# efeslab/Atom

Measured on AMD Instinct MI355X. Metric: effective TOPS, W4A4 group-128 GEMM + 128 INT8 outlier cols, fp16 out, higher is better.
Workload: dtype int4xint4 exact integer dot (BF6-coded on the f8f6f4 MFMA; INT8 MFMA for the keeper), fp32 dequant, fp16 out

## Files before the change

atom_amd/_lib.py:

```python
from __future__ import annotations

import ctypes
import os
import subprocess

_HERE = os.path.dirname(os.path.abspath(__file__))
LIB_PATH = os.path.join(_HERE, "libatom_hip.so")
CSRC = os.path.join(_HERE, "csrc")

OK = 0
ERR_INVALID_ARG, ERR_SHAPE, ERR_ALIGN, ERR_LAUNCH = -22, -33, -14, -5
SCALE_LAYOUT_REF = 0
SCALE_LAYOUT_PLAIN = 1
QUANT_KERNEL = 0
QUANT_SIM = 1
QUANT_WIDE_CODES = 0x100
A_WIDE = 0x100
QUANT_F6_CODES = 0x200
AB_F6 = 0x200
O4_REF_EXTREMA = 0x800
B_F6S = 0x400
WS_WEIGHT_CACHED = 0x1000
B_SCALE_PAIRS = 0x2000
WS_VERIFY = 0x4000
Q_REORDER, Q_RMSNORM, Q_ADD_RMSNORM, Q_SILU_MUL = 1, 2, 3, 4
KV_STEP_OVERFLOW, KV_STEP_BAD_LENGTH = 1, 2
KV_BEAM_BAD_PARENT, KV_BEAM_BAD_PAGE = 4, 8
GUIDE_FREE, GUIDE_DEAD = -1, -2
GUIDE_REJECTED, GUIDE_BAD_STATE = 1, 2
F6_PITCH = 104

_vp = ctypes.c_void_p
_i64 = ctypes.c_int64
_int = ctypes.c_int
_f32 = ctypes.c_float

SIGNATURES = {
    "atom_version": (ctypes.c_char_p, []),
    "atom_strerror": (ctypes.c_char_p, [_int]),
    "atom_scale_size": (ctypes.c_size_t, [_i64, _int]),
    "atom_gemm_w4a4_f16": (_int, [_vp] * 9 + [_i64, _i64, _i64, _int, _int, _int, _vp]),
    "atom_gemm_w4a4_workspace_bytes": (ctypes.c_size_t, [_i64, _i64, _i64]),
    "atom_gemm_w4a4_ws_recodes": (_int, [_i64, _i64, _i64]),
    "atom_gemm_w4a4_ws_recodes_cached": (_int, [_i64, _i64, _i64]),
    "atom_gemm_w4a4_packed_order": (_int, [_i64, _i64, _i64, _int]),
    "atom_check_scale_pairs": (_int, [_vp, _i64, _i64, _vp, _vp]),
    "atom_verify_weight_f6s": (_int, [_vp, _vp, _i64, _i64, _vp, _vp, _vp]),
    "atom_gemm_w4a4_f16_ws": (_int, [_vp] * 9 + [_i64, _i64, _i64, _int, _int, _int, _vp, ctypes.c_size_t, _vp]),
    "atom_gemm_w4a4_multi_fits": (_int, [_i64, _i64, _int, _i64]),
    "atom_gemm_w4a4_multi": (_int, [_vp] * 11 + [ctypes.c_uint, _vp, _i64, _i64, _int, _i64, _int, _int, _int, _vp]),
    "atom_gemm_w4a4_multi_q_fits": (_int, [_int, _i64, _i64, _int, _i64]),
    "atom_gemm_w4a4_multi_q": (_int, [_int] + [_vp] * 5 + [_f32, _f32] + [_vp] * 7 + [ctypes.c_uint, _vp, _i64, _i64, _int, _i64, _int, _int, _vp]),
    "atom_gemm_w4a4_o4": (_int, [_vp] * 10 + [_i64, _i64, _i64, _int, _int, _int, _vp]),
    "atom_gemm_w4a4_o4_workspace_bytes": (ctypes.c_size_t, [_i64, _i64, _i64]),
    "atom_gemm_w4a4_o4_ws": (_int, [_vp] * 10 + [_i64, _i64, _i64, _int, _int, _int, _vp, ctypes.c_size_t, _vp]),
    "atom_reorder_quant_f16": (_int, [_vp, _vp, _i64, _int, _int, _f32, _int, _vp, _vp, _vp, _vp, _vp, _vp]),
    "atom_rmsnorm_reorder_quant_f16": (_int, [_vp, _vp, _f32, _vp, _i64, _int, _int, _f32, _int,
                                              _vp, _vp, _vp, _vp, _vp, _vp]),
    "atom_add_rmsnorm_reorder_quant_f16": (_int, [_vp, _vp, _vp, _vp, _f32, _vp, _i64, _int, _int, _f32, _int,
                                                  _vp, _vp, _vp, _vp, _vp, _vp]),
    "atom_silu_mul_quant_f16": (_int, [_vp, _vp, _i64, _int, _int, _f32, _int, _vp, _vp, _vp, _vp, _vp, _vp]),
    "atom_quant_weight_w4": (_int, [_vp, _i64, _i64, _f32, _int, _vp, _vp, _vp, _vp, _vp, _vp]),
    "atom_pack_weight_w4": (_int, [_vp, _i64, _i64, _int, _vp, _vp, _vp, _vp, _vp, _vp]),
    "atom_f6_rows": (ctypes.c_size_t, [_i64]),
    "atom_repack_weight_f6": (_int, [_vp, _i64, _i64, _vp, _vp]),
    "atom_repack_act_f6": (_int, [_vp, _vp, _i64, _i64, _int, _vp, _vp]),
    "atom_f6_weight_bytes": (ctypes.c_size_t, [_i64, _i64]),
    "atom_gemm_w4a4_f6_order": (ctypes.c_int, [_i64, _i64, _i64]),
    "atom_repack_weight_f6s": (_int, [_vp, _vp, _i64, _i64, _vp, _vp]),
    "atom_kv_fake_quant_f16": (_int, [_vp, _vp, _i64, _int, _i64, _i64, _i64, _i64, _int, _f32, _vp]),
    "atom_kv_append_i4": (_int, [_vp] * 10 + [_i64] + [_int] * 6 + [_vp]),
    "atom_kv_quant_append_f32": (_int, [_vp] * 7 + [_int] * 6 + [_vp]),
    "atom_gemm_w4a4_f32": (_int, [_vp] * 9 + [_i64, _i64, _i64, _int, _int, _int, _vp]),
    "atom_gemm_w4a4_silu_mul_quant_f6": (_int, [_vp] * 6 + [_i64, _i64, _i64, _int, _int, _int, _f32, _int] + [_vp] * 6),
    "atom_batch_decode_i4_workspace_bytes": (ctypes.c_size_t, [_int, _int, _int, _int]),
    "atom_batch_decode_i4_splits": (_int, [_int, _int, _int, _int]),
    "atom_gemm_w4a4_multi_merge_q_fits": (_int, [_i64, _i64, _int, _i64, _int]),
    "atom_gemm_w4a4_multi_merge_q": (_int, [_vp, _int, _vp, _f32] + [_vp] * 7 + [ctypes.c_uint, _vp, _i64, _i64, _int, _i64, _int, _int, _vp]),
    "atom_batch_decode_i4": (_int, [_vp] * 7 + [_int] * 6 + [_f32, _f32, _int, _vp, ctypes.c_size_t, _vp]),
    "atom_batch_decode_append_i4": (_int, [_vp] * 9 + [_int] * 6 + [_f32, _f32, _int, _vp, ctypes.c_size_t, _vp]),
    "atom_batch_prefill_i4_workspace_bytes": (ctypes.c_size_t, [_i64, _int, _int, _int, _int, _int]),
    "atom_batch_prefill_i4": (_int, [_vp, _vp, _vp, _i64, _int] + [_vp] * 5 + [_int] * 6 + [_f32, _f32, _int, _vp, ctypes.c_size_t, _vp]),
    "atom_batch_decode_gqa_i4_workspace_bytes": (ctypes.c_size_t, [_int] * 5),
    "atom_batch_decode_gqa_i4_splits": (_int, [_int] * 5),
    "atom_batch_decode_gqa_i4": (_int, [_vp] * 7 + [_int] * 7 + [_f32, _f32, _int, _vp, ctypes.c_size_t, _vp]),
    "atom_batch_prefill_gqa_i4_workspace_bytes": (ctypes.c_size_t, [_i64] + [_int] * 6),
    "atom_batch_prefill_gqa_i4": (_int, [_vp, _vp, _vp, _i64, _int] + [_vp] * 5 + [_int] * 7 + [_f32, _f32, _int, _vp, ctypes.c_size_t, _vp]),
    "atom_kv_step_i4": (_int, [_vp] * 7 + [_int] * 4 + [_vp]),
    "atom_moe_max_tiles": (_i64, [_i64, _int]),
    "atom_moe_route_topk": (_int, [_vp, _i64, _int, _int] + [_vp] * 9),
    "atom_moe_gemm_w4a4_f16": (_int, [_vp] * 15 + [_i64, _i64, _int, _i64, _int, _i64, _int, _int, _int, _vp]),
# ... 66 lines not shown
```

atom_amd/csrc/common.h:

```cpp
#pragma once
#include <hip/hip_runtime.h>
#include <stdint.h>
#include <atomic>

#include "../../include/atom_hip.h"

#ifdef ATOM_TOOLS
#include <cstdlib>
#define ATOM_TUNE(name, dflt) ([]() -> int { const char *e = getenv(name); return e ? atoi(e) : (dflt); }())
#else
#define ATOM_TUNE(name, dflt) (dflt)
#endif

namespace atom {

constexpr int kGroup = 128;
constexpr int kKeeper = 128;

typedef _Float16 half_t;
typedef int v4i __attribute__((ext_vector_type(4)));
typedef int v16i __attribute__((ext_vector_type(16)));
typedef float v4f __attribute__((ext_vector_type(4)));
typedef unsigned int v4u __attribute__((ext_vector_type(4)));
typedef unsigned int v2u __attribute__((ext_vector_type(2)));
// ... 25 lines not shown
  float clip;
  int ref_layout;
};

struct GemmParams {
  const uint8_t *A4, *B4;
  const half_t *sA, *sB;
  const uint8_t *A8, *B8;
  const half_t *sA8, *sB8;
  half_t *D;
  uint8_t *D4;
  half_t *Dsz;
  float *ws;
  int splits;
  int M, N;
  int K4h;
  int G;
  int ref_layout;
  int a_wide;
  int64_t ldA;
  int64_t f6_rows_a, f6_rows_b;
  int o4_ref;
  int b_pairs;
  GateUpOut gu;
  const float *sB32;
  void *seg_out[3];
  const half_t *seg_add;
  int seg_n;
  unsigned seg_f32;
  int q_op;
  const half_t *q_x, *q_x2;
  const half_t *q_res;
  half_t *q_res_out;
  const int16_t *q_idx;
  float q_eps, q_clip;
  int q_roles;
  const float *q_part;
  int q_splits;
};

int launch_gemm_v2(const GemmParams &p, int ns, hipStream_t s);
int launch_gemm_v2_o4(const GemmParams &p, hipStream_t s);
int launch_gemm_v3(const GemmParams &p, int cfg, hipStream_t s);
int launch_gemv(const GemmParams &p, hipStream_t s);
#ifdef ATOM_TOOLS
constexpr int kGemvMaxTokens = 8;
#else
constexpr int kGemvMaxTokens = 2;
#endif
int launch_gemv1(const GemmParams &p, hipStream_t s);
int launch_gemv1_f32(const GemmParams &p, hipStream_t s);
int launch_gemv1_multi(const GemmParams &p, hipStream_t s);
int launch_gemm_skinny(const GemmParams &p, hipStream_t s);
int launch_gemm_skinny_f32(const GemmParams &p, hipStream_t s);
int launch_gemm_skinny_o4(const GemmParams &p, hipStream_t s);
int launch_gemm_skinny_multi(const GemmParams &p, hipStream_t s);
bool skinny_q_fits(int q_op, int64_t M, int64_t K_total);
int launch_gemm_skinny_multi_q(const GemmParams &p, hipStream_t s);
bool gemvq_fits(int q_op, int64_t M, int64_t N, int64_t K_total);
bool gemvq_merge_fits(int64_t M, int64_t N, int64_t K_total, int splits);
int launch_gemvq_multi_q(const GemmParams &p, hipStream_t s);
enum F6Cfg : int {
  F6_256x256 = 0, F6_128x128 = 3, F6_128x128_KG2 = 6, F6_256x128 = 8, F6_MID = 20,
  F6_256x128_P = 1, F6_64x128 = 2, F6_128x128_8W = 4, F6_128x128_KG2_S2 = 5, F6_64x128_KG2 = 9, F6_256x256_32 = 10, F6_64x128_KG4 = 12, F6_128x128_32 = 13, F6_256x256_P = 30,
};
inline int f6_cfg_order(int cfg) { return cfg == F6_64x128_KG4 ? 4 : ((cfg == F6_128x128_KG2_S2 || cfg == F6_128x128_KG2 || cfg == F6_64x128_KG2) ? 2 : 1); }
int launch_gemm_f6(const GemmParams &p, int cfg, hipStream_t s);
int launch_gemm_f6_mid(const GemmParams &p, hipStream_t s);
int launch_gemm_mid(const GemmParams &p, hipStream_t s);
int launch_gemm_f6_gateup(const GemmParams &p, int sim, hipStream_t s);

int launch_repack_f6(const uint8_t *src, int64_t rows, int K4h, int G, const half_t *scale, int64_t ld, int ref_layout,
                     uint8_t *out, hipStream_t s);
int launch_repack_f6_pair(const uint8_t *A4, int64_t M, const half_t *sA, int64_t ldA, int ref_layout, uint8_t *outA,
                          const half_t *sB, float *sB32,
                          const uint8_t *B4, int64_t N, uint8_t *outB, int K4h, int G, hipStream_t s);

int launch_check_scale_pairs(const half_t *sB, int64_t G, int64_t N, int32_t *n_bad, hipStream_t s);
int launch_verify_weight_f6s(const uint8_t *B4, const half_t *sB, int64_t N, int K4h, int G, const uint8_t *have, int32_t *n_bad, hipStream_t s);

template <int BYTES>
__device__ __forceinline__ void lds_dma(const void *gsrc, const void *lds_dst) {
  static_assert(BYTES == 16 || BYTES == 4 || BYTES == 2, "LDS-DMA piece size");
  const unsigned m0v = __builtin_amdgcn_readfirstlane((unsigned)(size_t)(const __attribute__((address_space(3))) char *)lds_dst);
  if constexpr (BYTES == 16) asm volatile("s_mov_b32 m0, %0\n\ts_nop 0\n\tglobal_load_lds_dwordx4 %1, off" ::"s"(m0v), "v"(gsrc) : "memory");
  else if constexpr (BYTES == 4) asm volatile("s_mov_b32 m0, %0\n\ts_nop 0\n\tglobal_load_lds_dword %1, off" ::"s"(m0v), "v"(gsrc) : "memory");
// ... 81 lines not shown
```

atom_amd/csrc/gemm_w4a4.hip:

```cpp
#include "common.h"

using namespace atom;

static bool shape_ok(int64_t M, int64_t N, int64_t K_total, bool n64) {
  return M >= 1 && N >= 64 && (!n64 || (N % 64) == 0) && K_total >= 256 && ((K_total - kKeeper) % kGroup) == 0;
}
static bool segments_ok(int64_t M, int64_t N_seg, int nseg, int64_t K_total) {
  return M >= 1 && nseg >= 1 && nseg <= 3 && N_seg >= 16 && (N_seg % 16) == 0 && K_total >= 256 && ((K_total - kKeeper) % kGroup) == 0;
}

static void fill_dims(GemmParams &p, int64_t M, int64_t N, int64_t K_total, int scale_layout, bool f6, bool f6s) {
  p.M = (int)M; p.N = (int)N;
  p.K4h = (int)((K_total - kKeeper) / 2); p.G = (int)((K_total - kKeeper) / kGroup);
  p.ref_layout = scale_layout == ATOM_SCALE_LAYOUT_REF;
  p.f6_rows_a = f6 ? (M + 255) / 256 * 256 : 0;
  p.f6_rows_b = f6 ? (N + 255) / 256 * 256 : 0;
  p.sB32 = f6s ? reinterpret_cast<const float *>(p.B4 + (size_t)p.G * (size_t)p.f6_rows_b * 104) : nullptr;
  p.ldA = (int64_t)atom_scale_size(M, scale_layout);
}

static int fill_params(GemmParams &p, const void *A4, const void *B4, const void *sA, const void *sB, const void *A8,
                       const void *B8, const void *sA8, const void *sB8, int64_t M, int64_t N, int64_t K_total, int group,
                       int keeper, int scale_layout) {
  if (!A4 || !B4 || !sA || !sB || !A8 || !B8 || !sA8 || !sB8) return ATOM_ERR_INVALID_ARG;
  const int a_wide = (scale_layout & ATOM_A_WIDE) != 0;
  const int f6 = (scale_layout & ATOM_AB_F6) != 0, f6s = (scale_layout & ATOM_B_F6S) != 0;
  p.o4_ref = (scale_layout & ATOM_O4_REF_EXTREMA) != 0;
  p.b_pairs = (scale_layout & ATOM_B_SCALE_PAIRS) != 0;
  scale_layout &= ~(ATOM_A_WIDE | ATOM_AB_F6 | ATOM_B_F6S | ATOM_O4_REF_EXTREMA | ATOM_WS_WEIGHT_CACHED | ATOM_B_SCALE_PAIRS | ATOM_WS_VERIFY);
  if ((a_wide && f6) || (f6s && !f6)) return ATOM_ERR_INVALID_ARG;
  if (scale_layout != ATOM_SCALE_LAYOUT_REF && scale_layout != ATOM_SCALE_LAYOUT_PLAIN) return ATOM_ERR_INVALID_ARG;
  if (group != kGroup || keeper != kKeeper) return ATOM_ERR_SHAPE;
  if (!shape_ok(M, N, K_total, true)) return ATOM_ERR_SHAPE;
  if (M > (1 << 24) || N > (1 << 24) || K_total > (1 << 20)) return ATOM_ERR_SHAPE;
  if ((M > N ? M : N) * ((K_total - kKeeper) / 2) >= (int64_t(1) << 32)) return ATOM_ERR_SHAPE;
  if (a_wide && M * (K_total - kKeeper) >= (int64_t(1) << 32)) return ATOM_ERR_SHAPE;
  if (!aligned16(A4) || !aligned16(B4) || !aligned16(A8) || !aligned16(B8)) return ATOM_ERR_ALIGN;
  if ((reinterpret_cast<uintptr_t>(sB) & 3u) || (reinterpret_cast<uintptr_t>(sB8) & 3u)) return ATOM_ERR_ALIGN;
  p.A4 = (const uint8_t *)A4; p.B4 = (const uint8_t *)B4;
  p.sA = (const half_t *)sA;  p.sB = (const half_t *)sB;
  p.A8 = (const uint8_t *)A8; p.B8 = (const uint8_t *)B8;
  p.sA8 = (const half_t *)sA8; p.sB8 = (const half_t *)sB8;
  p.D = nullptr; p.D4 = nullptr; p.Dsz = nullptr; p.ws = nullptr; p.splits = 1; p.q_op = 0; p.q_part = nullptr; p.q_splits = 0; p.q_roles = 0;
  p.a_wide = a_wide;
  fill_dims(p, M, N, K_total, scale_layout, f6, f6s);
  return ATOM_OK;
}

static int gemv_max_m() { return ATOM_TUNE("ATOM_GEMV_MAXM", 7); }
static int gemv_tokens(int64_t K_total) {
  const int forced = ATOM_TUNE("ATOM_GEMV_TOKENS", 0);
  const int t = forced > 0 ? forced : (K_total > 4096 ? 2 : 1);
// ... 83 lines not shown
  if (wide) return 20 + (cm256 * cn256 >= 128 ? 0 : small);
  if (cm256 * cn256 >= 1024) return 0;
  return cm256 * cn128 >= 512 ? 1 : small;
}

static int f6_pick_cfg(int64_t M, int64_t N, int64_t K_total) {
  const int force = ATOM_TUNE("ATOM_F6_CFG", -1);
  if (force >= 0) return force;
  const int64_t t256 = ((M + 255) / 256) * ((N + 255) / 256), t128 = ((M + 127) / 128) * ((N + 127) / 128);
  const int64_t rounds = (t256 + 255) / 256, steps = (K_total - kKeeper) / kGroup + 2;
  if ((N % 64) == 0 && ((M + 63) / 64) * (N / 64) <= 512 && ATOM_TUNE("ATOM_F6_MID", 1)) return F6_MID;
  if (t256 >= 129 && (rounds == 1 || 5 * t256 >= 3 * rounds * 256)) return F6_256x256;
#ifdef ATOM_TOOLS
  const int64_t t64 = ((M + 63) / 64) * ((N + 127) / 128);
  if (steps >= 16 && t64 <= 256) return F6_64x128_KG4;
  if (steps >= 8 && t64 <= 256) return F6_64x128_KG2;
#endif
  if (steps >= 8 && t128 <= 256) return F6_128x128_KG2;
  const int64_t t2 = ((M + 255) / 256) * ((N + 127) / 128);
  if (steps >= 6 && t2 > 128 && t2 <= 256 && ATOM_TUNE("ATOM_Q2", 1)) return F6_256x128;
  return F6_128x128;
}

struct RecodeWs { uint8_t *b6; float *sb32; uint8_t *a6; size_t bytes; };
static RecodeWs recode_ws(void *workspace, int64_t M, int64_t N, int64_t K_total) {
  const size_t G = (size_t)((K_total - kKeeper) / kGroup), wb = G * (size_t)((N + 255) / 256 * 256) * 104;
  uint8_t *b6 = (uint8_t *)workspace;
  return {b6, reinterpret_cast<float *>(b6 + wb), b6 + wb / 104 * 108, wb / 104 * 108 + G * (size_t)((M + 255) / 256 * 256) * 104};
}

static int verify_assertions(const GemmParams &p, int64_t M, int64_t N, int64_t K_total, int flags, void *workspace, size_t workspace_bytes,
                             hipStream_t hs) {
  if (!workspace || workspace_bytes < 16 || !aligned16(workspace)) return ATOM_ERR_INVALID_ARG;
  int32_t *cnt = reinterpret_cast<int32_t *>((uint8_t *)workspace + ((workspace_bytes - 16) & ~(size_t)15));
  if (hipMemsetAsync(cnt, 0, 16, hs) != hipSuccess) return ATOM_ERR_LAUNCH;
  if (p.b_pairs && !p.f6_rows_a) {
    const int r = launch_check_scale_pairs(p.sB, p.G, N, cnt, hs);
    if (r != ATOM_OK) return r;
  }
  if ((flags & ATOM_WS_WEIGHT_CACHED) && !p.a_wide && !p.f6_rows_a && packed_route(M, N, K_total, WS_WEIGHT_CACHED).kernel == K_RECODE) {
    if (workspace_bytes < atom_gemm_w4a4_workspace_bytes(M, N, K_total)) return ATOM_ERR_INVALID_ARG;
    const int r = launch_verify_weight_f6s(p.B4, p.sB, N, p.K4h, p.G, (const uint8_t *)workspace, cnt + 1, hs);
    if (r != ATOM_OK) return r;
  }
  int32_t host[2] = {0, 0};
  if (hipMemcpyAsync(host, cnt, sizeof(host), hipMemcpyDeviceToHost, hs) != hipSuccess || hipStreamSynchronize(hs) != hipSuccess)
// ... 15 lines not shown
  const int variant = ATOM_TUNE("ATOM_GEMM_VARIANT", 0);
  st = ATOM_ERR_INVALID_ARG;
  if (p.a_wide && variant != 0 && !(variant >= 320 && variant <= 330)) return true;
  if (p.f6_rows_a && variant != 0) return true;
  switch (variant) {
    case 203: case 2: case 204: st = launch_gemm_v2(p, variant == 203 ? 3 : 4, hs); return true;
    case 1001: case 1002: case 1003: case 1004: case 1008: case 1016: case 1019: case 1023: case 1031: case 1032: case 1033: case 1035: case 1064: case 1128: case 1256:
      st = launch_gemm_v2(p, variant, hs); return true;
    case 300: case 301: case 302: case 303: case 304: case 305: case 306: case 320: case 324: case 325:
      st = launch_gemm_v3(p, variant - 300, hs); return true;
    case 310: case 311: case 330:
      if ((p.Dsz = trace_ptr())) st = launch_gemm_v3(p, variant - 300, hs);
      return true;
    default: return false;
  }
}
#endif

static int run_plain(GemmParams &p, int64_t M, int64_t N, int64_t K_total, hipStream_t hs) {
#ifdef ATOM_TOOLS
  int st;
  if (run_variant(p, hs, st)) return st;
#endif
  if (p.f6_rows_a) return launch_gemm_f6(p, f6_pick_cfg(M, N, K_total), hs);
  if (p.a_wide) return launch_gemm_v3(p, tile_cfg(M, N, true), hs);
  return run_packed(p, packed_route(M, N, K_total, WS_NONE), hs);
}

static int check_segments(const void *out0, const void *out1, const void *out2, unsigned f32_mask, const void *add0_f16, int64_t N_seg,
                          int nseg, int scale_layout) {
  if (nseg < 1 || nseg > 3 || !out0 || (nseg > 1 && !out1) || (nseg > 2 && !out2)) return ATOM_ERR_INVALID_ARG;
  if (scale_layout & (ATOM_A_WIDE | ATOM_AB_F6)) return ATOM_ERR_INVALID_ARG;
  if (N_seg < 16 || (N_seg % 16) != 0) return ATOM_ERR_SHAPE;
  if ((f32_mask & 1u) && add0_f16) return ATOM_ERR_INVALID_ARG;
  return ATOM_OK;
}
static int fill_segments(GemmParams &p, void *out0, void *out1, void *out2, unsigned f32_mask, const void *add0_f16, int64_t N_seg) {
  if (!aligned16(out0) || (out1 && !aligned16(out1)) || (out2 && !aligned16(out2)) || (add0_f16 && !aligned16(add0_f16))) return ATOM_ERR_ALIGN;
  p.seg_out[0] = out0; p.seg_out[1] = out1; p.seg_out[2] = out2;
  p.seg_add = (const half_t *)add0_f16;
  p.seg_n = (int)N_seg;
  p.seg_f32 = f32_mask;
  return ATOM_OK;
}

extern "C" {

int atom_gemm_w4a4_f6_order(int64_t M, int64_t N, int64_t K_total) {
  return shape_ok(M, N, K_total, false) ? f6_cfg_order(f6_pick_cfg(M, N, K_total)) : 0;
}

const char *atom_version(void) { return "atom_hip 0.1 (gfx950)"; }

const char *atom_strerror(int code) {
  switch (code) {
    case ATOM_OK: return "ok";
    case ATOM_ERR_INVALID_ARG: return "invalid argument (null pointer or bad enum)";
    case ATOM_ERR_SHAPE: return "unsupported shape / group / keeper";
    case ATOM_ERR_ALIGN: return "pointer not 16-byte aligned";
    case ATOM_ERR_LAUNCH: return "HIP launch failed";
    default: return "unknown error";
  }
}

int atom_gemm_w4a4_f16(const void *A4, const void *B4, const void *sA, const void *sB, const void *A8,
                       const void *B8, const void *sA8, const void *sB8, void *D, int64_t M, int64_t N,
                       int64_t K_total, int group, int keeper, int scale_layout, void *stream) {
  return atom_gemm_w4a4_f16_ws(A4, B4, sA, sB, A8, B8, sA8, sB8, D, M, N, K_total, group, keeper, scale_layout & ~ATOM_WS_VERIFY, nullptr, 0, stream);
}

int atom_gemm_w4a4_packed_order(int64_t M, int64_t N, int64_t K_total, int with_workspace) {
  if (!shape_ok(M, N, K_total, true)) return 0;
// ... 32 lines not shown
  if (!D) return ATOM_ERR_INVALID_ARG;
  const size_t need = workspace ? atom_gemm_w4a4_workspace_bytes(M, N, K_total) : 0;
  const bool usable = need != 0 && workspace_bytes >= need;
  if (!aligned16(D) || (usable && (!aligned16(workspace) || (N % 8) != 0))) return ATOM_ERR_ALIGN;
  p.D = (half_t *)D;
  if (!usable) return run_plain(p, M, N, K_total, hs);
  if (p.f6_rows_a) {
#ifdef ATOM_TOOLS
    const int cfg = f6_pick_cfg(M, N, K_total), sp = ATOM_TUNE("ATOM_F6_SPLITS3", 0), most = workspace_splits(packed_route(M, N, K_total, WS_NONE), M, N, K_total, true);
    if (most > 1 && (cfg == F6_128x128 || cfg == F6_128x128_8W) && sp > 1 && sp <= most) { p.ws = (float *)workspace; p.splits = sp; }
    if (most > 1) return launch_gemm_f6(p, cfg, hs);
#endif
    return run_plain(p, M, N, K_total, hs);
  }
  const Route r = packed_route(M, N, K_total, (scale_layout & ATOM_WS_WEIGHT_CACHED) ? WS_WEIGHT_CACHED : WS_FREE);
  if (!p.a_wide && r.kernel == K_RECODE) {
    const RecodeWs w = recode_ws(workspace, M, N, K_total);
    const int rc = r.recode_weight
                       ? launch_repack_f6_pair(p.A4, M, p.sA, p.ldA, p.ref_layout, w.a6, p.sB, w.sb32, p.B4, N, w.b6, p.K4h, p.G, hs)
                       : launch_repack_f6(p.A4, M, p.K4h, p.G, p.sA, p.ldA, p.ref_layout, w.a6, hs);
    if (rc != ATOM_OK) return rc;
    p.A4 = w.a6; p.B4 = w.b6;
    fill_dims(p, M, N, K_total, p.ref_layout ? ATOM_SCALE_LAYOUT_REF : ATOM_SCALE_LAYOUT_PLAIN, true, true);
    return launch_gemm_f6(p, f6_pick_cfg(M, N, K_total), hs);
  }
  const int splits = p.a_wide ? workspace_splits(r, M, N, K_total, false) : (r.kernel == K_SPLITK ? r.splits : 1);
  if (splits <= 1) return run_plain(p, M, N, K_total, hs);
  p.ws = (float *)workspace; p.splits = splits;
  return launch_gemm_v3(p, tile_cfg(M, N, p.a_wide, splits), hs);
}

int atom_gemm_w4a4_o4(const void *A4, const void *B4, const void *sA, const void *sB, const void *A8, const void *B8,
                      const void *sA8, const void *sB8, void *D_u4, void *D_scale_zero, int64_t M, int64_t N,
                      int64_t K_total, int group, int keeper, int scale_layout, void *stream) {
  if (!D_u4 || !D_scale_zero) return ATOM_ERR_INVALID_ARG;
  GemmParams p;
  const int st = fill_params(p, A4, B4, sA, sB, A8, B8, sA8, sB8, M, N, K_total, group, keeper, scale_layout);
  if (st != ATOM_OK) return st;
  if ((N % 128) != 0) return ATOM_ERR_SHAPE;
  if (p.a_wide || p.f6_rows_a) return ATOM_ERR_INVALID_ARG;
  if (!aligned16(D_u4)) return ATOM_ERR_ALIGN;
  p.D4 = (uint8_t *)D_u4; p.Dsz = (half_t *)D_scale_zero;
  return launch_gemm_v2_o4(p, reinterpret_cast<hipStream_t>(stream));
}

int atom_gemm_w4a4_f32(const void *A4, const void *B4, const void *sA, const void *sB, const void *A8, const void *B8,
                       const void *sA8, const void *sB8, void *D_f32, int64_t M, int64_t N, int64_t K_total, int group,
// ... 162 lines not shown
```

atom_amd/csrc/gemm_w4a4_f6.hip:

```cpp
#include <type_traits>
#include "common.h"
#include "quant_math.h"

namespace atom {

__global__ void splitk_reduce_kernel(const float *ws, half_t *D, int64_t MN, int splits);

namespace f6 {

typedef const __attribute__((address_space(1))) void *gptr_t;
typedef __attribute__((address_space(3))) void *lptr_t;
typedef int v8i __attribute__((ext_vector_type(8)));
typedef float v16f __attribute__((ext_vector_type(16)));

constexpr int TN = 2;
constexpr int PITCH = 104;
constexpr float kMagic = 12582912.0f;
constexpr int kMagicBits = 0x4B400000;

template <int BM_, int BN_, int TM_, int NS_, int OCC_ = 2, int FS_ = 0>
struct Cfg {
  static constexpr int FS = FS_;
  static constexpr int FS32 = FS_ == 1;
  static constexpr int OCC = OCC_;
// ... 1710 lines not shown
          *reinterpret_cast<unsigned *>(d6 + 2) = (f[0] >> 16) | (f[1] << 16);
        }
        if (wn == 0 && kb == 0) *reinterpret_cast<v2u *>(dst + 96) = f6_scale_words(__builtin_bit_cast(unsigned short, sh));
      }
      if (wn == 0 && kb == 0) store_token_scale(keeper_blk ? o.s8 : (o.s4 + (int64_t)bn * o.ld4), m, sh, o.ref_layout);
      if (o.xq) {
        v4u q;
        half_t *qv = reinterpret_cast<half_t *>(&q);
#pragma unroll
        for (int j = 0; j < 8; ++j) qv[j] = dequant_half(tr[j], gs);
        *reinterpret_cast<v4u *>(o.xq + m * N_inter + bn * 128 + wn * 32 + kb * 8) = q;
      }
    }
    return;
  }
}

template <class C, int GU = 0, bool TR = false, bool PAIR = false>
static int launch_q(const GemmParams &p, hipStream_t s) {
  static std::atomic<uint64_t> attr_done{0};
  if (ensure_max_lds(reinterpret_cast<const void *>(&gemm_w4a4_f6q_kernel<C, GU, TR, PAIR>), QC<C>::LDS_BYTES, attr_done) != ATOM_OK) return ATOM_ERR_LAUNCH;
  const int nbm = (p.M + C::BM - 1) / C::BM, nbn = (p.N + C::BN - 1) / C::BN;
  hipLaunchKernelGGL((gemm_w4a4_f6q_kernel<C, GU, TR, PAIR>), dim3((unsigned)(nbm * nbn)), dim3(C::NT), QC<C>::LDS_BYTES, s, p);
  return check_launch();
}

struct QkDma {
  unsigned voff, voffX;
  int m0W, m0A, m0X;
  int xkind;
};
__device__ __forceinline__ void q_dma4(unsigned m0v, unsigned voff, const void *sbase) {
  asm volatile("s_mov_b32 m0, %0\n\ts_nop 0\n\tglobal_load_lds_dword %1, %2" ::"s"(m0v), "v"(voff), "s"(sbase) : "memory");
}
template <class C>
__device__ __forceinline__ void qk_piece(const QkDma &d, const uint8_t *wsrc, const uint8_t *asrc, const float *sbsrc, int so, int i) {
  if (i == 0) q_dma16x3(so + d.m0W, d.voff, wsrc);
  else if (i == 1) q_dma16x3(so + d.m0A, d.voff, asrc);
  else if (i == 2) {
    if (d.xkind == 3) q_dma4(so + d.m0X, d.voffX, sbsrc);
    else q_dma16(so + d.m0X, d.voffX, d.xkind == 1 ? (const void *)wsrc : (const void *)asrc);
  }
}

template <class C>
struct QkRegs {
// ... 554 lines not shown
#endif

int launch_gemm_f6(const GemmParams &p, int cfg, hipStream_t s) {
#ifdef ATOM_TOOLS
  int st;
  if (launch_gemm_f6_tools(p, cfg, s, st)) return st;
#endif
  if (cfg == F6_MID) {
    const int r = launch_gemm_f6_mid(p, s);
    if (r != ATOM_ERR_SHAPE) return r;
    cfg = F6_128x128;
  }
  if (cfg == F6_256x128) {
    if (p.sB32 && p.G >= 2) return f6::launch_q2<f6::Cfg<256, 128, 2, 3, 2, 1>>(p, s);
    cfg = F6_128x128;
  }
  if (cfg == F6_128x128)
    return f6_128_f32_scales(p) ? f6::launch_x16<f6::Cfg<128, 128, 2, 2, 3, 1>>(p, s) : f6::launch_x16<f6::Cfg<128, 128, 2, 2, 3, 2>>(p, s);
  if (cfg == F6_128x128_KG2) {
    if (p.sB32 && p.G >= 7 && ATOM_TUNE("ATOM_QK", 1)) return f6::launch_qk<f6::Cfg<128, 128, 2, 3, 3, 1>>(p, s);
    if (p.sB32) return f6::launch_x16<f6::Cfg<128, 128, 2, 3, 3, 1>, false, 2>(p, s);
    return f6::launch_x16<f6::Cfg<128, 128, 2, 3, 3, 2>, false, 2>(p, s);
  }
  if (!p.sB32) return f6::launch_p<f6::Cfg<256, 256, 4, 3>>(p, s);
  if (p.b_pairs) return f6::launch_q<f6::Cfg<256, 256, 4, 3>, 0, false, true>(p, s);
  return f6::launch_q<f6::Cfg<256, 256, 4, 3>>(p, s);
}

}
```

include/atom_hip.h:

```cpp
#ifndef ATOM_HIP_H_
#define ATOM_HIP_H_

#include <stddef.h>
#include <stdint.h>

#ifdef __cplusplus
extern "C" {
#endif

#define ATOM_OK 0
#define ATOM_ERR_INVALID_ARG (-22)
#define ATOM_ERR_SHAPE (-33)
#define ATOM_ERR_ALIGN (-14)
#define ATOM_ERR_LAUNCH (-5)

#define ATOM_SCALE_LAYOUT_REF 0
#define ATOM_SCALE_LAYOUT_PLAIN 1

#define ATOM_QUANT_KERNEL 0
#define ATOM_QUANT_SIM 1

#define ATOM_QUANT_WIDE_CODES 0x100
#define ATOM_A_WIDE 0x100

#define ATOM_QUANT_F6_CODES 0x200
#define ATOM_AB_F6 0x200
int atom_gemm_w4a4_f6_order(int64_t M, int64_t N, int64_t K_total);
#define ATOM_B_F6S 0x400
#define ATOM_O4_REF_EXTREMA 0x800
#define ATOM_WS_WEIGHT_CACHED 0x1000
#define ATOM_B_SCALE_PAIRS 0x2000
#define ATOM_WS_VERIFY 0x4000
#define ATOM_F6_PITCH 104

const char *atom_version(void);
const char *atom_strerror(int code);

size_t atom_scale_size(int64_t rows, int scale_layout);

int atom_gemm_w4a4_f16(const void *A4, const void *B4, const void *sA, const void *sB,
                       const void *A8, const void *B8, const void *sA8, const void *sB8,
                       void *D, int64_t M, int64_t N, int64_t K_total,
                       int group, int keeper, int scale_layout, void *stream);

size_t atom_gemm_w4a4_workspace_bytes(int64_t M, int64_t N, int64_t K_total);
int atom_gemm_w4a4_ws_recodes(int64_t M, int64_t N, int64_t K_total);
int atom_gemm_w4a4_ws_recodes_cached(int64_t M, int64_t N, int64_t K_total);
int atom_check_scale_pairs(const void *sB, int64_t G, int64_t N, int32_t *n_bad_dev, void *stream);
int atom_verify_weight_f6s(const void *B4, const void *sB, int64_t N, int64_t K_total, const void *B_f6s, int32_t *n_bad_dev, void *stream);
int atom_gemm_w4a4_f16_ws(const void *A4, const void *B4, const void *sA, const void *sB,
                          const void *A8, const void *B8, const void *sA8, const void *sB8,
                          void *D, int64_t M, int64_t N, int64_t K_total,
                          int group, int keeper, int scale_layout,
                          void *workspace, size_t workspace_bytes, void *stream);
int atom_gemm_w4a4_packed_order(int64_t M, int64_t N, int64_t K_total, int with_workspace);
// ... 205 lines not shown
```

Measured before the change: 2804.

## Add opt-in 16-wave 256x256 F6 GEMM kernel selected by Q16 flag

Adds a new 256x256 tile F6 GEMM kernel with 16 waves of 64x64 each (1024 threads), a three-stage LDS pipeline, and a fused INT8 keeper epilogue. The goal is more waves per tile so latency is hidden better than in the existing 4-wave 256x256 path. The kernel runs only when the caller sets the new ATOM_F6_Q16 layout flag, because the automatic heuristic returns false. It also adds a geometry query API. The default path is unchanged unless the benchmark passes the flag.

```diff
diff --git a/atom_amd/_lib.py b/atom_amd/_lib.py
--- a/atom_amd/_lib.py
+++ b/atom_amd/_lib.py
@@ -21,6 +21,7 @@
 O4_REF_EXTREMA = 0x800
 B_F6S = 0x400
 WS_WEIGHT_CACHED = 0x1000
+F6_Q16 = 0x8000
 B_SCALE_PAIRS = 0x2000
 WS_VERIFY = 0x4000
 Q_REORDER, Q_RMSNORM, Q_ADD_RMSNORM, Q_SILU_MUL = 1, 2, 3, 4
@@ -67,6 +68,7 @@
     "atom_repack_act_f6": (_int, [_vp, _vp, _i64, _i64, _int, _vp, _vp]),
     "atom_f6_weight_bytes": (ctypes.c_size_t, [_i64, _i64]),
     "atom_gemm_w4a4_f6_order": (ctypes.c_int, [_i64, _i64, _i64]),
+    "atom_gemm_w4a4_f6_geometry": (ctypes.c_int, [_i64, _i64, _i64, ctypes.c_int]),
     "atom_repack_weight_f6s": (_int, [_vp, _vp, _i64, _i64, _vp, _vp]),
     "atom_kv_fake_quant_f16": (_int, [_vp, _vp, _i64, _int, _i64, _i64, _i64, _i64, _int, _f32, _vp]),
     "atom_kv_append_i4": (_int, [_vp] * 10 + [_i64] + [_int] * 6 + [_vp]),
diff --git a/atom_amd/csrc/common.h b/atom_amd/csrc/common.h
--- a/atom_amd/csrc/common.h
+++ b/atom_amd/csrc/common.h
@@ -71,6 +71,7 @@
   int64_t f6_rows_a, f6_rows_b;
   int o4_ref;
   int b_pairs;
+  int f6_q16;
   GateUpOut gu;
   const float *sB32;
   void *seg_out[3];
@@ -111,6 +112,7 @@
 int launch_gemvq_multi_q(const GemmParams &p, hipStream_t s);
 enum F6Cfg : int {
   F6_256x256 = 0, F6_128x128 = 3, F6_128x128_KG2 = 6, F6_256x128 = 8, F6_MID = 20,
+  F6_256x256_Q16 = 16,
   F6_256x128_P = 1, F6_64x128 = 2, F6_128x128_8W = 4, F6_128x128_KG2_S2 = 5, F6_64x128_KG2 = 9, F6_256x256_32 = 10, F6_64x128_KG4 = 12, F6_128x128_32 = 13, F6_256x256_P = 30,
 };
 inline int f6_cfg_order(int cfg) { return cfg == F6_64x128_KG4 ? 4 : ((cfg == F6_128x128_KG2_S2 || cfg == F6_128x128_KG2 || cfg == F6_64x128_KG2) ? 2 : 1); }
diff --git a/atom_amd/csrc/gemm_w4a4.hip b/atom_amd/csrc/gemm_w4a4.hip
--- a/atom_amd/csrc/gemm_w4a4.hip
+++ b/atom_amd/csrc/gemm_w4a4.hip
@@ -27,7 +27,8 @@
   const int f6 = (scale_layout & ATOM_AB_F6) != 0, f6s = (scale_layout & ATOM_B_F6S) != 0;
   p.o4_ref = (scale_layout & ATOM_O4_REF_EXTREMA) != 0;
   p.b_pairs = (scale_layout & ATOM_B_SCALE_PAIRS) != 0;
-  scale_layout &= ~(ATOM_A_WIDE | ATOM_AB_F6 | ATOM_B_F6S | ATOM_O4_REF_EXTREMA | ATOM_WS_WEIGHT_CACHED | ATOM_B_SCALE_PAIRS | ATOM_WS_VERIFY);
+  p.f6_q16 = (scale_layout & ATOM_F6_Q16) != 0;
+  scale_layout &= ~(ATOM_A_WIDE | ATOM_AB_F6 | ATOM_B_F6S | ATOM_O4_REF_EXTREMA | ATOM_WS_WEIGHT_CACHED | ATOM_B_SCALE_PAIRS | ATOM_WS_VERIFY | ATOM_F6_Q16);
   if ((a_wide && f6) || (f6s && !f6)) return ATOM_ERR_INVALID_ARG;
   if (scale_layout != ATOM_SCALE_LAYOUT_REF && scale_layout != ATOM_SCALE_LAYOUT_PLAIN) return ATOM_ERR_INVALID_ARG;
   if (group != kGroup || keeper != kKeeper) return ATOM_ERR_SHAPE;
@@ -157,6 +158,22 @@
   return F6_128x128;
 }
 
+static bool f6_q16_faster(int64_t M, int64_t N, int64_t K_total) {
+  (void)M; (void)N; (void)K_total;
+  return false;
+}
+static bool f6_q16_fits(bool f6s, bool pairs, int64_t N, int64_t K_total) {
+  return f6s && pairs && (K_total - kKeeper) / kGroup >= 6 && N <= (1 << 21);
+}
+static int f6_cfg_for(int64_t M, int64_t N, int64_t K_total, bool f6s, bool pairs, bool ask_q16) {
+  const int cfg = f6_pick_cfg(M, N, K_total);
+  if (ATOM_TUNE("ATOM_F6_CFG", -1) >= 0 || cfg != F6_256x256 || !f6_q16_fits(f6s, pairs, N, K_total)) return cfg;
+  return ask_q16 || f6_q16_faster(M, N, K_total) ? F6_256x256_Q16 : cfg;
+}
+static int f6_cfg_of(const GemmParams &p, int64_t M, int64_t N, int64_t K_total) {
+  return f6_cfg_for(M, N, K_total, p.sB32 != nullptr, p.b_pairs != 0, p.f6_q16 != 0);
+}
+
 struct RecodeWs { uint8_t *b6; float *sb32; uint8_t *a6; size_t bytes; };
 static RecodeWs recode_ws(void *workspace, int64_t M, int64_t N, int64_t K_total) {
   const size_t G = (size_t)((K_total - kKeeper) / kGroup), wb = G * (size_t)((N + 255) / 256 * 256) * 104;
@@ -218,7 +235,7 @@
   int st;
   if (run_variant(p, hs, st)) return st;
 #endif
-  if (p.f6_rows_a) return launch_gemm_f6(p, f6_pick_cfg(M, N, K_total), hs);
+  if (p.f6_rows_a) return launch_gemm_f6(p, f6_cfg_of(p, M, N, K_total), hs);
   if (p.a_wide) return launch_gemm_v3(p, tile_cfg(M, N, true), hs);
   return run_packed(p, packed_route(M, N, K_total, WS_NONE), hs);
 }
@@ -244,6 +261,11 @@
 
 int atom_gemm_w4a4_f6_order(int64_t M, int64_t N, int64_t K_total) {
   return shape_ok(M, N, K_total, false) ? f6_cfg_order(f6_pick_cfg(M, N, K_total)) : 0;
+}
+
+int atom_gemm_w4a4_f6_geometry(int64_t M, int64_t N, int64_t K_total, int scale_layout) {
+  if (!shape_ok(M, N, K_total, true)) return -1;
+  return f6_cfg_for(M, N, K_total, (scale_layout & ATOM_B_F6S) != 0, (scale_layout & ATOM_B_SCALE_PAIRS) != 0, (scale_layout & ATOM_F6_Q16) != 0);
 }
 
 const char *atom_version(void) { return "atom_hip 0.1 (gfx950)"; }
@@ -322,7 +344,7 @@
     if (rc != ATOM_OK) return rc;
     p.A4 = w.a6; p.B4 = w.b6;
     fill_dims(p, M, N, K_total, p.ref_layout ? ATOM_SCALE_LAYOUT_REF : ATOM_SCALE_LAYOUT_PLAIN, true, true);
-    return launch_gemm_f6(p, f6_pick_cfg(M, N, K_total), hs);
+    return launch_gemm_f6(p, f6_cfg_of(p, M, N, K_total), hs);
   }
   const int splits = p.a_wide ? workspace_splits(r, M, N, K_total, false) : (r.kernel == K_SPLITK ? r.splits : 1);
   if (splits <= 1) return run_plain(p, M, N, K_total, hs);
diff --git a/atom_amd/csrc/gemm_w4a4_f6.hip b/atom_amd/csrc/gemm_w4a4_f6.hip
--- a/atom_amd/csrc/gemm_w4a4_f6.hip
+++ b/atom_amd/csrc/gemm_w4a4_f6.hip
@@ -1756,6 +1756,287 @@
   if (ensure_max_lds(reinterpret_cast<const void *>(&gemm_w4a4_f6q_kernel<C, GU, TR, PAIR>), QC<C>::LDS_BYTES, attr_done) != ATOM_OK) return ATOM_ERR_LAUNCH;
   const int nbm = (p.M + C::BM - 1) / C::BM, nbn = (p.N + C::BN - 1) / C::BN;
   hipLaunchKernelGGL((gemm_w4a4_f6q_kernel<C, GU, TR, PAIR>), dim3((unsigned)(nbm * nbn)), dim3(C::NT), QC<C>::LDS_BYTES, s, p);
+  return check_launch();
+}
+
+template <class C>
+struct Q16Regs {
+  v8i af[2];
+  v8i bf[2];
+  float sb[4];
+  float sa[4];
+  v4f_t acc[2];
+  int aW[2], aA[2], aS[2], aB[2];
+};
+
+template <class C, int SL>
+__device__ __forceinline__ v8i q16_frag(const int (&a)[2], int off, int ro) {
+  const int b = a[q_set<SL>()] + (SL < 0 ? ro : 0), imm = q_imm<C, SL>() + off;
+  const v2u x = q_ld0<v2u>(b, imm);
+  asm volatile("" ::: "memory");
+  const v2u y = q_ld0<v2u>(b, imm + 8);
+  asm volatile("" ::: "memory");
+  const v2u z = q_ld0<v2u>(b, imm + 16);
+  asm volatile("" ::: "memory");
+  return v8i{(int)x.x, (int)x.y, (int)y.x, (int)y.y, (int)z.x, (int)z.y, 0, 0};
+}
+template <class C, int SL>
+__device__ __forceinline__ float q16_sa(const Q16Regs<C> &R, int tb, int ro) {
+  return q_ld0<float>(R.aS[q_set<SL>()] + (SL < 0 ? ro : 0), q_imm<C, SL>() + p_row(tb) * PITCH);
+}
+template <class C, int SL>
+__device__ __forceinline__ void q16_sb(Q16Regs<C> &R, int h, int ro) {
+#pragma unroll
+  for (int r = 0; r < 4; ++r) {
+    R.sb[r] = q_ld0<float>(R.aB[q_set<SL>()] + (SL < 0 ? ro : 0), q_imm<C, SL>() + 128 * h + 8 * r);
+    asm volatile("" ::: "memory");
+  }
+}
+
+struct Q16Dma {
+  unsigned voff;
+  int m0, m0X;
+  int xkind;
+  int xadj;
+};
+template <class C, int DS>
+__device__ __forceinline__ void q16_piece(const Q16Dma &d, const uint8_t *src, const float *sbsrc, int i) {
+  constexpr int base = DS * QC<C>::STAGE;
+  if (i == 0) q_dma16x3(base + d.m0, d.voff, src);
+  else if (i == 1 && d.xkind != 0)
+    q_dma16(base + d.m0X, d.voff, (d.xkind == 1 ? src : reinterpret_cast<const uint8_t *>(sbsrc)) + d.xadj);
+}
+
+struct QNoKeep { __device__ __forceinline__ void operator()() const {} };
+__device__ __forceinline__ int q16_lane() {
+  int l = (int)__builtin_amdgcn_mbcnt_hi(~0u, __builtin_amdgcn_mbcnt_lo(~0u, 0u));
+  asm volatile("" : "+v"(l));
+  return l;
+}
+template <class C, int SL, class FS, class FD, class FE, class FK = QNoKeep>
+__device__ __forceinline__ void q16_step(Q16Regs<C> &R, float (&c)[4][4][4], FS sync, FD mid, FE early, bool last, FK keep = FK(), int ro = 0, int rn = 0) {
+  constexpr int NX = SL < 0 ? -1 : (SL + 1) % 3;
+#pragma unroll
+  for (int i = 0; i < 8; ++i) {
+    const int tb = i & 3, h = i >> 2;
+    __builtin_amdgcn_sched_barrier(0);
+    if (i == 4) sync();
+    __builtin_amdgcn_sched_barrier(0);
+#pragma unroll
+    for (int k = 0; k < 2; ++k)
+      R.acc[k] = __builtin_amdgcn_mfma_scale_f32_16x16x128_f8f6f4(R.af[k], R.bf[tb & 1], v4f_t{0.f, 0.f, 0.f, 0.f}, 3, 3, 0, 0, 0, 0);
+    __builtin_amdgcn_sched_barrier(0);
+    if (i < 6) R.bf[tb & 1] = q16_frag<C, SL>(R.aA, p_row((i + 2) & 3) * PITCH, ro);
+    else if (!last) R.bf[tb & 1] = q16_frag<C, NX>(R.aA, p_row((i + 2) & 3) * PITCH, rn);
+    if (i == 3) {
+      R.af[0] = q16_frag<C, SL>(R.aW, p_row(2) * PITCH, ro);
+      R.af[1] = q16_frag<C, SL>(R.aW, p_row(3) * PITCH, ro);
+    }
+    if (i == 7 && !last) {
+      R.af[0] = q16_frag<C, NX>(R.aW, p_row(0) * PITCH, rn);
+      R.af[1] = q16_frag<C, NX>(R.aW, p_row(1) * PITCH, rn);
+    }
+    if (i >= 4) mid(i - 4);
+    else early(i);
+    __builtin_amdgcn_sched_barrier(0);
+    deq_pair<true>(R.acc[0], R.acc[1], R.sa[tb], R.sb, c[2 * h][tb], c[2 * h + 1][tb]);
+    __builtin_amdgcn_sched_barrier(0);
+    if (i == 3) q16_sb<C, SL>(R, 1, ro);
+    if (i == 4) { keep(); __builtin_amdgcn_sched_barrier(0); }
+    if (i >= 4 && !last) R.sa[tb] = q16_sa<C, NX>(R, tb, rn);
+    if (i == 7 && !last) q16_sb<C, NX>(R, 0, rn);
+  }
+}
+
+template <class C>
+__device__ __forceinline__ void q16_keeper(const GemmParams &p, const char *slot, const char *slot1, int wm, int wn, int lane, float (&c)[4][4][4],
+                                           int m0, int n0) {
+  const int l15 = lane & 15, kb = lane >> 4;
+  const int sw = (l15 >> 1) & 3;
+  const char *pw = slot + (wn * 64 + 2 * l15) * 64 + ((kb ^ sw) << 4);
+  const char *pa = slot + (C::BN + wm * 64 + 2 * l15) * 64 + ((kb ^ sw) << 4);
+  const char *psa = slot + C::KP_SA_OFF + (wm * 64 + 2 * l15) * 4;
+  const char *psb = slot + C::SB_OFF + (wn * 64 + 8 * kb) * 2;
+  const long d1 = slot1 - slot;
+  unsigned dvoff = 0;
+  auto store_block = [&](int tb) {
+    const int ln = q16_lane();
+    if (m0 + wm * 64 + p_row(tb) + 2 * (ln & 15) >= p.M) return;
+    char *dtb = reinterpret_cast<char *>(p.D + ((int64_t)(m0 + p_row(tb)) * p.N + n0));
+#pragma unroll
+    for (int h = 0; h < 2; ++h) {
+      if (n0 + wn * 64 + 32 * h + 8 * (ln >> 4) >= p.N) continue;
+      v4u o;
+      half_t *ov = reinterpret_cast<half_t *>(&o);
+#pragma unroll
+      for (int r = 0; r < 4; ++r) {
+        ov[2 * r] = f2h(c[2 * h][tb][r]);
+        ov[2 * r + 1] = f2h(c[2 * h + 1][tb][r]);
+      }
+      *reinterpret_cast<v4u *>(dtb + dvoff + 64 * h) = o;
+    }
+  };
+#pragma unroll
+  for (int h = 0; h < 2; ++h) {
+    if (h == 1) {
+      const int ln = q16_lane();
+      dvoff = (unsigned)(((wm * 64 + 2 * (ln & 15)) * p.N + wn * 64 + 8 * (ln >> 4)) * 2);
+      asm volatile("" : "+v"(dvoff));
+    }
+    const v4u sbw = *reinterpret_cast<const v4u *>(psb + 64 * h);
+#pragma unroll
+    for (int tb = 0; tb < 4; ++tb) {
+      __builtin_amdgcn_sched_barrier(0);
+      if (h == 1 && tb >= 1) store_block(tb - 1);
+      const float sa = (float)*reinterpret_cast<const half_t *>(psa + p_row(tb) * 4);
+      const half_t *hv = reinterpret_cast<const half_t *>(&sbw);
+#pragma unroll
+      for (int k = 0; k < 2; ++k) {
+        v4i acc;
+#pragma unroll
+        for (int r = 0; r < 4; ++r) { int m = kMagicBits; asm volatile("" : "+v"(m)); acc[r] = m; }
+#pragma unroll
+        for (int half = 0; half < 2; ++half) {
+          __builtin_amdgcn_sched_barrier(0);
+          const long dh = half ? d1 : 0;
+          const v4i bf = __builtin_bit_cast(v4i, *reinterpret_cast<const v4u *>(pa + dh + p_row(tb) * 64));
+          const v4i af = __builtin_bit_cast(v4i, *reinterpret_cast<const v4u *>(pw + dh + p_row(2 * h + k) * 64));
+          acc = __builtin_amdgcn_mfma_i32_16x16x64_i8(af, bf, acc, 0, 0, 0);
+        }
+        __builtin_amdgcn_sched_barrier(0);
+        float t[4];
+#pragma unroll
+        for (int r = 0; r < 4; ++r) {
+          float w = (float)hv[2 * r + k];
+          asm volatile("" : "+v"(w));
+          t[r] = sa * w;
+        }
+#pragma unroll
+        for (int r = 0; r < 4; ++r) {
+          c[2 * h + k][tb][r] = __builtin_fmaf(__int_as_float(acc[r]) - kMagic, t[r], c[2 * h + k][tb][r]);
+          asm volatile("" : "+v"(c[2 * h + k][tb][r]));
+        }
+      }
+    }
+  }
+  store_block(3);
+}
+
+template <class C>
+__global__ __launch_bounds__(1024, 1) void gemm_w4a4_f6q16_kernel(GemmParams p) {
+  extern __shared__ __attribute__((aligned(16))) char lds[];
+  static_assert(C::BM == 256 && C::BN == 256 && C::WM == 64 && C::NS == 3 && C::NW == 16, "q16 kernel: 256x256, 16 waves of 64 x 64");
+  using Q = QC<C>;
+  const int tid = threadIdx.x;
+  const int lane = tid & 63;
+  const int wave = __builtin_amdgcn_readfirstlane(tid >> 6);
+  __builtin_assume(wave >= 0 && wave < C::NW);
+  const int wm = wave >> 2, wn = wave & 3;
+  const int nbn = (p.N + C::BN - 1) / C::BN, nbm = (p.M + C::BM - 1) / C::BM;
+  const int nwg = nbm * nbn;
+  int id = blockIdx.x;
+  {
+    const int q = nwg >> 3, r = nwg & 7, xcd = id & 7, k = id >> 3;
+    id = (xcd < r ? xcd * (q + 1) : r * (q + 1) + (xcd - r) * q) + k;
+  }
+  constexpr int GM = 4;
+  const int band = id / (GM * nbn), inband = id % (GM * nbn);
+  const int rows_in_band = min(GM, nbm - band * GM);
+  const int bm = band * GM + inband % rows_in_band, bn = inband / rows_in_band;
+  const int m0 = bm * C::BM, n0 = bn * C::BN;
+
+  float c[4][4][4];
+#pragma unroll
+  for (int a = 0; a < 4; ++a)
+#pragma unroll
+    for (int b = 0; b < 4; ++b)
+#pragma unroll
+      for (int r = 0; r < 4; ++r) c[a][b][r] = 0.f;
+
+  const int G = p.G;
+  Q16Dma d;
+  const int chunk = wave >> 2, first = 13 * (chunk & 1) + 3 * (wave & 3);
+  d.voff = (unsigned)(first * 1024 + lane * 16);
+  d.m0 = (13 * chunk + 3 * (wave & 3)) * 1024;
+  d.xkind = (wave & 3) == 0 ? 1 : (wave == 1 ? 3 : 0);
+  d.m0X = wave == 1 ? Q::SB_OFF : (13 * chunk + 12) * 1024;
+  d.xadj = wave == 1 ? -first * 1024 : 12 * 1024;
+  const bool isw = chunk < 2;
+  const int64_t ostep = (isw ? p.f6_rows_b : p.f6_rows_a) * PITCH;
+  const uint8_t *src0 = isw ? p.B4 + (int64_t)n0 * PITCH : p.A4 + (int64_t)m0 * PITCH;
+  const float *sbsrc0 = p.sB32 + n0;
+  auto slot_of = [&](int stage) { return lds + (stage % 3) * Q::STAGE; };
+#pragma unroll
+  for (int i = 0; i < 2; ++i) q16_piece<C, 0>(d, src0, sbsrc0, i);
+  asm volatile("s_waitcnt vmcnt(0)" ::: "memory");
+  __builtin_amdgcn_s_barrier();
+
+  const int l15 = lane & 15, kb = lane >> 4;
+  Q16Regs<C> R;
+  {
+    const int lw = wn * 64 * PITCH + l15 * (2 * PITCH) + kb * 24;
+    const int la = C::A_OFF + wm * 64 * PITCH + l15 * (2 * PITCH);
+#pragma unroll
+    for (int st = 0; st < 2; ++st) {
+      R.aW[st] = lw + st * 2 * Q::STAGE;
+      R.aA[st] = la + kb * 24 + st * 2 * Q::STAGE;
+      R.aS[st] = la + 100 + st * 2 * Q::STAGE;
+      R.aB[st] = Q::SB_OFF + (wn * 64 + 8 * kb) * 4 + st * 2 * Q::STAGE;
+      asm volatile("" : "+v"(R.aW[st]), "+v"(R.aA[st]), "+v"(R.aS[st]), "+v"(R.aB[st]));
+    }
+    R.bf[0] = q16_frag<C, 0>(R.aA, p_row(0) * PITCH, 0);
+    R.af[0] = q16_frag<C, 0>(R.aW, p_row(0) * PITCH, 0);
+    R.af[1] = q16_frag<C, 0>(R.aW, p_row(1) * PITCH, 0);
+    R.bf[1] = q16_frag<C, 0>(R.aA, p_row(1) * PITCH, 0);
+#pragma unroll
+    for (int tb = 0; tb < 4; ++tb) R.sa[tb] = q16_sa<C, 0>(R, tb, 0);
+    q16_sb<C, 0>(R, 1, 0);
+    if (wm & 1) {
+#pragma unroll
+      for (int r = 0; r < 4; ++r) c[2][3][r] = c[3][3][r] = __builtin_fmaf(0.f, 0.f * R.sb[r], 0.f);
+    }
+    q16_sb<C, 0>(R, 0, 0);
+  }
+  auto sync = [&]() {
+    asm volatile("s_waitcnt vmcnt(0)" ::: "memory");
+    __builtin_amdgcn_s_barrier();
+  };
+  auto reg = [&](auto sl, int s) {
+    constexpr int SL = decltype(sl)::value;
+    const uint8_t *src = src0 + (s + 2) * ostep;
+    const float *sbsrc = sbsrc0 + (int64_t)(s + 2) * p.f6_rows_b;
+    q16_step<C, SL>(R, c, sync, [&](int i) { q16_piece<C, (SL + 2) % 3>(d, src, sbsrc, i); }, QNoEarly(), false);
+  };
+  using S0 = std::integral_constant<int, 0>;
+  using S1 = std::integral_constant<int, 1>;
+  using S2 = std::integral_constant<int, 2>;
+  q16_step<C, 0>(R, c, sync, [&](int i) { q16_piece<C, 2>(d, src0 + 2 * ostep, sbsrc0 + (int64_t)2 * p.f6_rows_b, i); },
+                 [&](int i) { q16_piece<C, 1>(d, src0 + ostep, sbsrc0 + p.f6_rows_b, i); }, false);
+  reg(S1(), 1);
+  reg(S2(), 2);
+  int s = 3;
+  for (; s + 4 < G; s += 3) { reg(S0(), s); reg(S1(), s + 1); reg(S2(), s + 2); }
+  if (s + 2 < G) { reg(S0(), s); ++s; }
+  if (s + 2 < G) { reg(S1(), s); ++s; }
+  for (; s < G; ++s) {
+    q16_step<C, -1>(R, c, sync, QNoEarly(), QNoEarly(), s + 1 == G,
+                    [&]() {
+                      const int ln = q16_lane();
+                      issue_keeper<C>(p, s + 2 - G, slot_of(s + 2), wave, ln, m0, n0);
+                    },
+                    (s % 3) * Q::STAGE, ((s + 1) % 3) * Q::STAGE);
+  }
+  asm volatile("s_waitcnt vmcnt(0)" ::: "memory");
+  __builtin_amdgcn_s_barrier();
+  q16_keeper<C>(p, slot_of(G), slot_of(G + 1), wm, wn, q16_lane(), c, m0, n0);
+}
+
+template <class C>
+static int launch_q16(const GemmParams &p, hipStream_t s) {
+  static std::atomic<uint64_t> attr_done{0};
+  if (ensure_max_lds(reinterpret_cast<const void *>(&gemm_w4a4_f6q16_kernel<C>), QC<C>::LDS_BYTES, attr_done) != ATOM_OK) return ATOM_ERR_LAUNCH;
+  const int nbm = (p.M + C::BM - 1) / C::BM, nbn = (p.N + C::BN - 1) / C::BN;
+  hipLaunchKernelGGL((gemm_w4a4_f6q16_kernel<C>), dim3((unsigned)(nbm * nbn)), dim3(C::NT), QC<C>::LDS_BYTES, s, p);
   return check_launch();
 }
 
@@ -2356,6 +2637,8 @@
     if (p.sB32) return f6::launch_x16<f6::Cfg<128, 128, 2, 3, 3, 1>, false, 2>(p, s);
     return f6::launch_x16<f6::Cfg<128, 128, 2, 3, 3, 2>, false, 2>(p, s);
   }
+  if (cfg == F6_256x256_Q16 && p.sB32 && p.b_pairs && p.G >= 6 && p.N <= (1 << 21))
+    return f6::launch_q16<f6::Cfg<256, 256, 2, 3, 4>>(p, s);
   if (!p.sB32) return f6::launch_p<f6::Cfg<256, 256, 4, 3>>(p, s);
   if (p.b_pairs) return f6::launch_q<f6::Cfg<256, 256, 4, 3>, 0, false, true>(p, s);
   return f6::launch_q<f6::Cfg<256, 256, 4, 3>>(p, s);
diff --git a/include/atom_hip.h b/include/atom_hip.h
--- a/include/atom_hip.h
+++ b/include/atom_hip.h
@@ -31,6 +31,8 @@
 #define ATOM_WS_WEIGHT_CACHED 0x1000
 #define ATOM_B_SCALE_PAIRS 0x2000
 #define ATOM_WS_VERIFY 0x4000
+#define ATOM_F6_Q16 0x8000
+int atom_gemm_w4a4_f6_geometry(int64_t M, int64_t N, int64_t K_total, int scale_layout);
 #define ATOM_F6_PITCH 104
 
 const char *atom_version(void);
```

Result: slower. 2746 (-2.1%).
